# mumianyuxin/M3DSSD

Measured on AMD Instinct MI355X. Metric: images/sec at 1280x384 bs=8, 1/2/4/8 MI355X; 3D-box Linf vs ref, higher is better.
Workload: dtype f32; 1 GPU; BASELINE.json configs[1]: full M3d_inference_align (DLA-34 + DCNv2 align + ANAB) forward + decode + top-3000 + NMS, bs=8/GPU, 1280x384, fp32, random-init synthetic weights and frames; per_gpu_batch=8, global_batch=8, parallelism=dp1 (batch sharded, 1 all-gather of [B,40,14] detections)

## Files before the change

### include/m3dssd_hip.h

```cpp
#ifndef M3DSSD_HIP_H
#define M3DSSD_HIP_H

#include <stdint.h>

#ifdef __cplusplus
extern "C" {
#endif

typedef void *m3d_stream_t;

enum {
    M3D_OK = 0,
    M3D_E_ARG = -1,
    M3D_E_HIP = -2,
    M3D_E_WORKSPACE = -3
};

const char *m3d_last_error(void);
#define M3D_ABI_VERSION 5
int m3d_abi_version(void);
const char *m3d_source_hashes(void);

typedef struct m3d_conv_desc {
    const float *in;
// ... 15 lines not shown
    int res_mode;
    int act;
    int sigmoid_from;
    const float *dcn_offmask;
    int dcn_om_cs;
    float *splitk_ws;
    long long splitk_ws_bytes;
} m3d_conv_desc;

int m3d_conv2d_forward(const m3d_conv_desc *d, m3d_stream_t stream);
int m3d_conv2d_splitk_plan(const m3d_conv_desc *d, int *splits, long long *ws_bytes);

int m3d_conv_wave_applicable(const m3d_conv_desc *d);
int m3d_conv_wave_splitk_plan(const m3d_conv_desc *d, int *splits, long long *ws_bytes);
int m3d_conv_wave_forward(const m3d_conv_desc *d, m3d_stream_t stream);

int m3d_wino_conv3x3_forward(const m3d_conv_desc *d, m3d_stream_t stream);
int m3d_wino_conv3x3_variant(const m3d_conv_desc *d);
int m3d_wino_conv3x3_splitk_plan(const m3d_conv_desc *d, int *splits, long long *ws_bytes);
int m3d_wino_conv3x3_forward_ex(const m3d_conv_desc *d, int variant, m3d_stream_t stream);
int m3d_wino44_applicable(const m3d_conv_desc *d);
int m3d_wino44_conv3x3_forward(const m3d_conv_desc *d, m3d_stream_t stream);
int m3d_wino44_conv3x3_forward_ex(const m3d_conv_desc *d, int nb, m3d_stream_t stream);
int m3d_wino44_kpair(const m3d_conv_desc *d);
int m3d_wino44_splitk_plan(const m3d_conv_desc *d, int *splits, long long *ws_bytes);
int m3d_wino44_conv3x3_forward_touch(const m3d_conv_desc *d, int nb, const void *touch, long long touch_bytes, m3d_stream_t stream);

int m3d_cache_touch(const void *p, long long bytes, m3d_stream_t stream);
int m3d_upload_indirect(const void *const *src_slot, void *dst, long long bytes, m3d_stream_t stream);

// ... 315 lines not shown
```

### m3dssd_amd/_hip.py

```python
import ctypes
import os
import subprocess

_HERE = os.path.dirname(os.path.abspath(__file__))
CSRC = os.path.join(_HERE, "csrc")
SO_PATH = os.environ.get("M3D_HIP_LIB") or os.path.join(CSRC, "build", "libm3dssd_hip.so")
HEADER = os.path.join(os.path.dirname(_HERE), "include", "m3dssd_hip.h")

c_int, c_float, c_ll, c_void_p = ctypes.c_int, ctypes.c_float, ctypes.c_longlong, ctypes.c_void_p


class ConvDesc(ctypes.Structure):
    _fields_ = [
        ("inp", c_void_p), ("in_cs", c_int),
        ("N", c_int), ("H", c_int), ("W", c_int), ("Cin", c_int),
        ("wgt", c_void_p), ("wgt_img_stride", c_ll),
        ("Cout", c_int), ("Cout_pad", c_int),
        ("kh", c_int), ("kw", c_int), ("stride", c_int), ("pad", c_int), ("dil", c_int),
        ("Ho", c_int), ("Wo", c_int),
        ("out", c_void_p), ("out_cs", c_int), ("out_nchw", c_int), ("out_img_stride", c_ll),
        ("scale", c_void_p), ("shift", c_void_p),
        ("res", c_void_p), ("res_cs", c_int), ("res_mode", c_int),
        ("act", c_int), ("sigmoid_from", c_int),
        ("dcn_offmask", c_void_p), ("dcn_om_cs", c_int),
# ... 111 lines not shown
    "m3d_wino_conv3x3_forward": (c_int, [ctypes.POINTER(ConvDesc), P]),
    "m3d_wino_conv3x3_forward_ex": (c_int, [ctypes.POINTER(ConvDesc), c_int, P]),
    "m3d_wino_conv3x3_splitk_plan": (c_int, [ctypes.POINTER(ConvDesc), ctypes.POINTER(c_int), ctypes.POINTER(c_ll)]),
    "m3d_wino_conv3x3_variant": (c_int, [ctypes.POINTER(ConvDesc)]),
    "m3d_wino44_applicable": (c_int, [ctypes.POINTER(ConvDesc)]),
    "m3d_wino44_conv3x3_forward": (c_int, [ctypes.POINTER(ConvDesc), P]),
    "m3d_wino44_conv3x3_forward_ex": (c_int, [ctypes.POINTER(ConvDesc), c_int, P]),
    "m3d_wino44_kpair": (c_int, [ctypes.POINTER(ConvDesc)]),
    "m3d_wino44_conv3x3_forward_touch": (c_int, [ctypes.POINTER(ConvDesc), c_int, P, c_ll, P]),
    "m3d_cache_touch": (c_int, [P, c_ll, P]),
    "m3d_upload_indirect": (c_int, [P, P, c_ll, P]),
    "m3d_wino44_splitk_plan": (c_int, [ctypes.POINTER(ConvDesc), ctypes.POINTER(c_int), ctypes.POINTER(c_ll)]),
    "m3d_conv_wave_applicable": (c_int, [ctypes.POINTER(ConvDesc)]),
    "m3d_conv_wave_splitk_plan": (c_int, [ctypes.POINTER(ConvDesc), ctypes.POINTER(c_int), ctypes.POINTER(c_ll)]),
    "m3d_conv_wave_forward": (c_int, [ctypes.POINTER(ConvDesc), P]),
    "m3d_conv2d_tile": (c_int, [ctypes.POINTER(ConvDesc)] + [ctypes.POINTER(c_int)] * 4),
    "m3d_conv2d_splitk_plan": (c_int, [ctypes.POINTER(ConvDesc), ctypes.POINTER(c_int), ctypes.POINTER(c_ll)]),
    "m3d_dcn_v2_workspace_bytes": (c_ll, [c_int] * 10),
    "m3d_dcn_v2_workspace_bytes_grouped": (c_ll, [c_int] * 11),
    "m3d_dcn_v2_forward": (c_int, [P] * 6 + [c_int] * 14 + [P, c_ll, P]),
    "m3d_dcn_v2_backward_workspace_bytes": (c_ll, [c_int] * 11),
    "m3d_dcn_v2_backward": (c_int, [P] * 10 + [c_int] * 14 + [P, c_ll, P]),
    "m3d_rpn_loss_workspace_bytes": (c_ll, [c_int, c_ll]),
    "m3d_rpn_targets": (c_int, [P, c_int, c_int, c_int, P, c_int, P, c_int, c_int, P, P, c_int, P, P, P, P, P, c_ll, P]),
    "m3d_rpn_loss": (c_int, [P, c_int, c_int, c_int, P, c_int, P, c_int, c_int, P, P, P, c_int, P, P, P, P, P, P, P, P, P, P, c_ll, P]),
    "m3d_pack_conv_weight": (c_int, [P, P] + [c_int] * 6 + [P]),
    "m3d_nchw_to_nhwc": (c_int, [P, P] + [c_int] * 5 + [P]),
    "m3d_nhwc_to_nchw": (c_int, [P, c_int, P] + [c_int] * 4 + [P]),
    "m3d_stem_conv7x7": (c_int, [P, P, P, P, P] + [c_int] * 4 + [P]),
    "m3d_refine_3d": (c_int, [P, P, c_int, c_int, P, P, ctypes.c_double, c_int, ctypes.c_double, ctypes.c_double, P, P]),
# ... 92 lines not shown
```

### m3dssd_amd/csrc/common.h

```cpp
#pragma once
#include <hip/hip_runtime.h>
#include <stdarg.h>
#include <stdio.h>

#include "m3dssd_hip.h"

typedef float f32x4 __attribute__((ext_vector_type(4)));
typedef float f32x16 __attribute__((ext_vector_type(16)));
typedef float f32x2 __attribute__((ext_vector_type(2)));
typedef unsigned u32x4 __attribute__((ext_vector_type(4)));

__device__ __forceinline__ int sign_smear(int x)
{
    int m;
    asm("v_ashrrev_i32 %0, 31, %1" : "=v"(m) : "v"(x));
    return m;
}
__device__ __forceinline__ void dcn_corners(float h_im, float w_im, int H, int W, int drop_all, float (&w)[4], int (&o)[4],
                                            int (&drop)[4])
{
    const float tin = fminf(fminf(h_im, w_im) + 1.f, -fmaxf(h_im - (float)H, w_im - (float)W));
    const unsigned xin = __float_as_uint(tin);
    const unsigned nonfinite = __float_as_uint((h_im - h_im) + (w_im - w_im)) & 0x7fffffffu;
    const int out = sign_smear((int)((xin - 1u) | xin)) | sign_smear(-(int)nonfinite) | drop_all;
// ... 91 lines not shown
    do {                                                                            \
        hipError_t e__ = hipGetLastError();                                         \
        if (e__ != hipSuccess) {                                                    \
            m3d_set_error("kernel launch failed: %s (%s:%d)", hipGetErrorString(e__), \
                          __FILE__, __LINE__);                                      \
            return M3D_E_HIP;                                                       \
        }                                                                           \
    } while (0)

static inline int cdiv(long long a, long long b) { return (int)((a + b - 1) / b); }
static inline int imin(int a, int b) { return a < b ? a : b; }

__device__ __forceinline__ float leaky(float v) { return fmaxf(v, v * M3D_LEAKY_SLOPE); }
__device__ __forceinline__ float sigmoidf_(float v) { return 1.0f / (1.0f + expf(-v)); }

__device__ __forceinline__ f32x4 class_softmax4(f32x4 l)
{
    const float mx = fmaxf(fmaxf(l[0], l[1]), fmaxf(l[2], l[3]));
    f32x4 e;
    float s = 0.f;
#pragma unroll
    for (int c = 0; c < 4; ++c) { e[c] = expf(l[c] - mx); s += e[c]; }
    f32x4 pr;
#pragma unroll
    for (int c = 0; c < 4; ++c) pr[c] = e[c] / s;
    return pr;
}
__device__ __forceinline__ float fg_score(f32x4 pr) { return fmaxf(fmaxf(pr[1], pr[2]), pr[3]); }
__device__ __forceinline__ unsigned int f32_sortable(float f)
{
// ... 11 lines not shown
```

### m3dssd_amd/csrc/dcn_wave.hip

```cpp
#include <stdlib.h>

#include <type_traits>

#include "common.h"

struct ConvWaveArgs {
    const float *in, *wfrag, *scale, *shift, *res, *om;
    float *out;
    int in_cs, out_cs, res_cs, om_cs;
    int H, W, Cin, Ho, Wo, HoWo, Cout;
    int kh, kw, stride, pad, dil;
    int M, KG, tiles_n;
    int act, res_mode, sigmoid_from;
    int vec_out;
    long long w_img_stride;
    unsigned in_bytes, out_bytes, res_bytes, w_bytes;
    float *ws;
    int splits, ss_per, base_waves;
    unsigned ws_bytes;
#ifdef CONV_TRACE
    long long *trace;
#endif
};


#ifdef CONV_TRACE
static long long *g_conv_trace = nullptr;
extern "C" void m3d_conv_wave_set_trace(void *buf) { g_conv_trace = (long long *)buf; }
static int g_conv_variant = 0;
extern "C" void m3d_conv_wave_set_variant(int v) { g_conv_variant = v; }
#define TRACE_INIT() long long *trp = a.trace ? a.trace + (size_t)blockIdx.x * 128 : nullptr; int tri = 0
#define TRACE() do { if (trp && lane == 0 && tri < 128) trp[tri++] = __builtin_readcyclecounter(); } while (0)
#else
#define TRACE_INIT()
#define TRACE()
#endif

template <bool DEFORM, int NT, int NCQ = 4, int WPE = (DEFORM ? 2 : 3)>
__global__ __launch_bounds__(64) __attribute__((amdgpu_waves_per_eu(WPE))) void conv_wave_kernel(const ConvWaveArgs a)
{
    __shared__ __attribute__((aligned(16))) float tileA[32 * 32];
    __shared__ __attribute__((aligned(16))) float tapst[(DEFORM ? 9 : 1) * 32 * 8];
    const int lane = threadIdx.x, l31 = lane & 31, h = lane >> 5;
    const int gp = lane >> 3, gc = lane & 7;
    TRACE_INIT();
    TRACE();
    int blk;
    {
        const int nblk = gridDim.x, bid = blockIdx.x;
        const int q = nblk >> 3, r = nblk & 7, xcd = bid & 7, loc = bid >> 3;
        blk = (xcd < r ? xcd * (q + 1) : r * (q + 1) + (xcd - r) * q) + loc;
    }
    int split = 0;
    if (a.splits > 1) {
        split = blk / a.base_waves;
        blk -= split * a.base_waves;
    }
    const int bm = blk / a.tiles_n, bn = blk - bm * a.tiles_n;
    const int m0 = bm * 32;
    const int KK = a.kh * a.kw, C32 = a.Cin / 32;
    const int ss0 = split * a.ss_per, ss1 = min(KK * C32, ss0 + a.ss_per);

    const __amdgpu_buffer_rsrc_t rin = make_rsrc(a.in, a.in_bytes);
    const __amdgpu_buffer_rsrc_t rw =
        make_rsrc(a.wfrag + (size_t)(m0 / a.HoWo) * a.w_img_stride + (size_t)bn * NT * a.KG * 256, a.w_bytes);
    const unsigned wlane = (unsigned)lane * 16u;
    const unsigned wstride = (unsigned)a.KG * 1024u;

    int o_pix = 0, o_hi0 = 0, o_wi0 = 0;
    bool o_valid = false;
    int o_inv = -1;
    const float *o_om = a.om;
    int g_pix[4], g_hi0[4], g_wi0[4];
    bool g_valid[4];
    {
        const int m = m0 + l31;
// ... 12 lines not shown
        for (int g = 0; g < 4; ++g) {
            const int m = m0 + 8 * g + gp;
            g_valid[g] = m < a.M;
            const int mm = g_valid[g] ? m : 0;
            const int n = mm / a.HoWo, rem = mm - n * a.HoWo;
            const int ho = rem / a.Wo, wo = rem - ho * a.Wo;
            g_pix[g] = n * a.H * a.W;
            g_hi0[g] = ho * a.stride - a.pad;
            g_wi0[g] = wo * a.stride - a.pad;
        }
    }

    unsigned doff[4][DEFORM ? 4 : 1];
    float bw[DEFORM ? 4 : 1][4];
    if constexpr (DEFORM) {
        float raws[9][3];
#pragma unroll
        for (int t = 0; t < 9; ++t) {
            const int tp = min(t, KK - 1);
            raws[t][0] = o_om[2 * tp];
            raws[t][1] = o_om[2 * tp + 1];
            raws[t][2] = o_om[2 * KK + tp];
        }
#pragma unroll
        for (int t = 0; t < 9; ++t) {
            if (t < KK) {
                const int ti = t / a.kw, tj = t - ti * a.kw;
                const float mk = raws[t][2];
                const float h_im = (float)(o_hi0 + ti * a.dil) + raws[t][0];
                const float w_im = (float)(o_wi0 + tj * a.dil) + raws[t][1];
                float wq[4];
                int oq[4], drop[4];
                dcn_corners(h_im, w_im, a.H, a.W, o_inv, wq, oq, drop);
                u32x4 ob;
#pragma unroll
                for (int q = 0; q < 4; ++q) {
                    const unsigned off = ((unsigned)o_pix + (unsigned)oq[q]) * (unsigned)a.in_cs * 4u;
                    ob[q] = (off & ~(unsigned)drop[q]) | (M3D_BUF_OOB & (unsigned)drop[q]);
                }
                if (h == 0) {
                    *reinterpret_cast<u32x4 *>(&tapst[t * 256 + l31 * 8]) = ob;
                    *reinterpret_cast<f32x4 *>(&tapst[t * 256 + l31 * 8 + 4]) = f32x4{wq[0] * mk, wq[1] * mk, wq[2] * mk, wq[3] * mk};
                }
            }
        }
    }
    auto setup_tap = [&](int tap) {
        if constexpr (DEFORM) {
#pragma unroll
            for (int g = 0; g < 4; ++g) {
                const u32x4 ov = *reinterpret_cast<const u32x4 *>(&tapst[tap * 256 + (8 * g + gp) * 8]);
                const f32x4 wv = *reinterpret_cast<const f32x4 *>(&tapst[tap * 256 + (8 * g + gp) * 8 + 4]);
#pragma unroll
                for (int q = 0; q < 4; ++q) {
                    doff[g][q] = ov[q] + (unsigned)gc * 16u;
                    bw[g][q] = wv[q];
                }
            }
        } else {
            const int ti = tap / a.kw, tj = tap - ti * a.kw;
// ... 89 lines not shown
                for (int nt = 0; nt < NT; ++nt)
                    acc[nt] = __builtin_amdgcn_mfma_f32_32x32x2f32(A[j][t], bf[nt][t], acc[nt], 0, 0, 0);
            __builtin_amdgcn_sched_barrier(0);
        };
        group(0, kg0 + 1, bfA, bfB);
        group(1, kg0 + 2, bfB, bfA);
        group(2, kg0 + 3, bfA, bfB);
        group(3, kgn, bfB, bfA);
    }

    TRACE();
    const __amdgpu_buffer_rsrc_t rout = make_rsrc(a.out, a.out_bytes);
    const __amdgpu_buffer_rsrc_t rres = make_rsrc(a.res ? a.res : a.out, a.res ? a.res_bytes : 0u);
    const int n0 = bn * 32 * NT;
    const int mb = m0 + 4 * h;
    if (a.splits > 1) {
        const __amdgpu_buffer_rsrc_t rws = make_rsrc(a.ws, a.ws_bytes);
        const unsigned sbase = (unsigned)split * (unsigned)a.M;
        const unsigned cpad = (unsigned)(a.tiles_n * 32 * NT);
#pragma unroll
        for (int nt = 0; nt < NT; ++nt) {
            const unsigned co = (unsigned)(n0 + nt * 32 + l31);
#pragma unroll
            for (int r = 0; r < 16; ++r) {
                const int m = mb + (r & 3) + 8 * (r >> 2);
                const unsigned oo = m < a.M ? ((sbase + (unsigned)m) * cpad + co) * 4u : M3D_BUF_OOB;
                const float pv = acc[nt][r];
                __builtin_amdgcn_raw_buffer_store_b32(__builtin_bit_cast(unsigned, pv), rws, oo, 0, 0);
            }
        }
// ... 38 lines not shown
                        rv[q] = __builtin_bit_cast(f32x4, __builtin_amdgcn_raw_buffer_load_b128(rres, rq[q] + (unsigned)c * 4u, 0, 0));
                    } else {
#pragma unroll
                        for (int e = 0; e < 4; ++e)
                            rv[q][e] = __builtin_bit_cast(float, __builtin_amdgcn_raw_buffer_load_b32(
                                rres, c + e < a.Cout ? rq[q] + (unsigned)(c + e) * 4u : M3D_BUF_OOB, 0, 0));
                    }
                }
            }
#pragma unroll
            for (int r = 0; r < 16; ++r) tileA[((r & 3) + 8 * (r >> 2) + 4 * h) * 32 + l31] = acc[nt][r];
            const bool tile_sig = a.sigmoid_from >= 0 && n0 + nt * 32 + 31 >= a.sigmoid_from;
#pragma unroll
            for (int q = 0; q < 4; ++q) {
                f32x4 v = *reinterpret_cast<const f32x4 *>(&tileA[(pr + 8 * q) * 32 + 4 * c4]);
                if (a.res) v = a.res_mode ? (v + rv[q]) * scv[nt] + shv[nt] : v * scv[nt] + shv[nt] + rv[q];
                else v = v * scv[nt] + shv[nt];
                if (tile_sig) {
#pragma unroll
                    for (int e = 0; e < 4; ++e) v[e] = c + e >= a.sigmoid_from ? sigmoidf_(v[e]) : fmaxf(v[e], v[e] * slope);
                } else {
                    v = __builtin_elementwise_max(v, v * slope);
                }
                if (c + 3 < a.Cout) {
                    __builtin_amdgcn_raw_buffer_store_b128(__builtin_bit_cast(u32x4, v), rout, oq[q] + (unsigned)c * 4u, 0, 0);
                } else {
#pragma unroll
                    for (int e = 0; e < 4; ++e)
                        __builtin_amdgcn_raw_buffer_store_b32(__builtin_bit_cast(unsigned, v[e]), rout,
                                                              c + e < a.Cout ? oq[q] + (unsigned)(c + e) * 4u : M3D_BUF_OOB, 0, 0);
                }
            }
        }
        TRACE();
        return;
    }
#pragma unroll
    for (int nt = 0; nt < NT; ++nt) {
        const int co = n0 + nt * 32 + l31;
        const bool cok = co < a.Cout;
        const float sc = (cok && a.scale) ? a.scale[co] : 1.f;
        const float sh = (cok && a.shift) ? a.shift[co] : 0.f;
        float rv[16];
        if (a.res) {
#pragma unroll
            for (int r = 0; r < 16; ++r) {
                const int m = mb + (r & 3) + 8 * (r >> 2);
                const unsigned ro = (cok && m < a.M) ? ((unsigned)m * (unsigned)a.res_cs + (unsigned)co) * 4u : M3D_BUF_OOB;
                rv[r] = __builtin_bit_cast(float, __builtin_amdgcn_raw_buffer_load_b32(rres, ro, 0, 0));
            }
        }
#pragma unroll
        for (int r = 0; r < 16; ++r) {
            const int m = mb + (r & 3) + 8 * (r >> 2);
            float v = acc[nt][r];
            if (a.res) v = a.res_mode ? (v + rv[r]) * sc + sh : v * sc + sh + rv[r];
            else v = v * sc + sh;
            if (a.sigmoid_from >= 0 && co >= a.sigmoid_from) v = sigmoidf_(v);
            else if (a.act == 1) v = fmaxf(v, v * M3D_LEAKY_SLOPE);
            const unsigned oo = (cok && m < a.M) ? ((unsigned)m * (unsigned)a.out_cs + (unsigned)co) * 4u : M3D_BUF_OOB;
            __builtin_amdgcn_raw_buffer_store_b32(__builtin_bit_cast(unsigned, v), rout, oo, 0, 0);
        }
    }
    TRACE();
}

static int conv_wave_plan(const m3d_conv_desc *d, bool enforce_min, int *splits, int *ss_per)
{
    *splits = 1;
    *ss_per = d->kh * d->kw * (d->Cin / 32);
    if (d->out_nchw) return 0;
    if (d->dcn_offmask && d->kh * d->kw > 9) return 0;
    if (d->Cin % 32 != 0 || d->Cout_pad % 64 != 0) return 0;
    const int cw = d->Cout_pad % 128 == 0 ? 128 : 64;
    if (d->wgt_img_stride && (d->Ho * d->Wo) % 32 != 0) return 0;
    const long long M = (long long)d->N * d->Ho * d->Wo;
    const long long base = ((M + 31) / 32) * (d->Cout_pad / cw);
    if (base >= (1ll << 28)) return 0;
    static int wave_min = -1, dcn_min = -1, splitk = -1;
    if (wave_min < 0) { const char *e = getenv("M3D_CONV_WAVE_MIN"); wave_min = e ? atoi(e) : 900; }
    if (dcn_min < 0) { const char *e = getenv("M3D_DCN_WAVE_MIN"); dcn_min = e ? atoi(e) : 1500; }
    if (splitk < 0) { const char *e = getenv("M3D_CONV_WAVE_SPLITK"); splitk = e ? atoi(e) : 1; }
    const long long need = d->dcn_offmask ? dcn_min : wave_min;
    const int nss = *ss_per;
    if (base < need && splitk && d->splitk_ws) {
        int s = (int)((1800 + base - 1) / base);
        if (s > nss / 4) s = nss / 4;
        if (s > 8) s = 8;
        if (s >= 2) {
// ... 6 lines not shown
}

extern "C" int m3d_conv_wave_applicable(const m3d_conv_desc *d)
{
    int s, p;
    return d ? conv_wave_plan(d, true, &s, &p) : 0;
}

extern "C" int m3d_conv_wave_splitk_plan(const m3d_conv_desc *d, int *splits, long long *ws_bytes)
{
    M3D_REQUIRE(d && splits && ws_bytes, "conv_wave_splitk_plan: null pointer");
    m3d_conv_desc t = *d;
    static float dummy;
    t.splitk_ws = &dummy;
    int p;
    const int waves = conv_wave_plan(&t, true, splits, &p);
    if (waves == 0) *splits = 1;
    *ws_bytes = *splits > 1 ? (long long)*splits * d->N * d->Ho * d->Wo * d->Cout_pad * 4 : 0;
    return M3D_OK;
}

extern "C" int m3d_conv_wave_forward(const m3d_conv_desc *d, m3d_stream_t stream_)
{
    hipStream_t stream = (hipStream_t)stream_;
    M3D_REQUIRE(d && d->in && d->wgt && d->out, "conv_wave: null pointer");
    int splits = 1, ss_per = 0;
    const int waves = conv_wave_plan(d, false, &splits, &ss_per);
    M3D_REQUIRE(waves > 0, "conv_wave: needs Cin %% 32 == 0, Cout_pad %% 64 == 0, NHWC output, Ho*Wo %% 32 == 0 with per-image weights");
    const int ho = (d->H + 2 * d->pad - (d->dil * (d->kh - 1) + 1)) / d->stride + 1;
    const int wo = (d->W + 2 * d->pad - (d->dil * (d->kw - 1) + 1)) / d->stride + 1;
    M3D_REQUIRE(ho == d->Ho && wo == d->Wo, "conv_wave: Ho/Wo mismatch");
    M3D_REQUIRE(d->in_cs % 32 == 0 && d->in_cs >= d->Cin && ((uintptr_t)d->in & 127) == 0 && ((uintptr_t)d->wgt & 15) == 0,
                "conv_wave: the input view must be 128-byte aligned with in_cs %% 32 == 0");
    const long long M = (long long)d->N * d->Ho * d->Wo;
    M3D_REQUIRE(!d->wgt_img_stride || (d->wgt_img_stride % 4 == 0 && d->stride == 1 && d->Ho == d->H && d->Wo == d->W),
                "conv_wave: per-image weights need an image-aligned 16-byte stride and a same-size output");
    M3D_REQUIRE((long long)d->N * d->H * d->W * d->in_cs * 4 < (1ll << 31) && M * d->out_cs * 4 < (1ll << 31) &&
                M * d->res_cs * 4 < (1ll << 31) && (long long)d->Cout_pad * d->kh * d->kw * d->Cin * 4 < (1ll << 31),
                "conv_wave: views must be < 2 GiB");
    ConvWaveArgs a;
    a.in = d->in; a.wfrag = d->wgt; a.scale = d->scale; a.shift = d->shift; a.res = d->res; a.om = d->dcn_offmask;
    a.out = d->out;
    a.in_cs = d->in_cs; a.out_cs = d->out_cs; a.res_cs = d->res_cs; a.om_cs = d->dcn_om_cs;
    a.H = d->H; a.W = d->W; a.Cin = d->Cin; a.Ho = d->Ho; a.Wo = d->Wo; a.HoWo = d->Ho * d->Wo; a.Cout = d->Cout;
    a.kh = d->kh; a.kw = d->kw; a.stride = d->stride; a.pad = d->pad; a.dil = d->dil;
    const int cw = d->Cout_pad % 128 == 0 ? 128 : 64;
    a.M = (int)M; a.KG = d->kh * d->kw * d->Cin / 8; a.tiles_n = d->Cout_pad / cw;
    a.act = d->act; a.res_mode = d->res_mode; a.sigmoid_from = d->sigmoid_from; a.w_img_stride = d->wgt_img_stride;
    static int vec_epi = -1;
    if (vec_epi < 0) { const char *e = getenv("M3D_WAVE_VEC_EPILOGUE"); vec_epi = e ? atoi(e) : 1; }
    a.vec_out = vec_epi && d->out_cs % 4 == 0 && ((uintptr_t)d->out & 15) == 0 &&
                (!d->res || (d->res_cs % 4 == 0 && ((uintptr_t)d->res & 15) == 0)) &&
                (!d->scale || ((uintptr_t)d->scale & 15) == 0) && (!d->shift || ((uintptr_t)d->shift & 15) == 0);
    a.in_bytes = (unsigned)((long long)d->N * d->H * d->W * d->in_cs * 4);
    a.out_bytes = (unsigned)(M * d->out_cs * 4);
    a.res_bytes = (unsigned)(M * d->res_cs * 4);
    a.w_bytes = (unsigned)((long long)cw * d->kh * d->kw * d->Cin * 4);
#ifdef CONV_TRACE
    a.trace = g_conv_trace;
#endif
    a.ws = nullptr; a.splits = 1; a.ss_per = ss_per; a.base_waves = waves; a.ws_bytes = 0;
    if (splits > 1) {
        const long long need = (long long)splits * M * d->Cout_pad * 4;
        M3D_REQUIRE(need <= d->splitk_ws_bytes && need < (1ll << 31) && ((uintptr_t)d->splitk_ws & 15) == 0,
                    "conv_wave: split-K workspace too small (%lld bytes, see m3d_conv_wave_splitk_plan), >= 2 GiB or misaligned",
                    d->splitk_ws_bytes);
        a.ws = d->splitk_ws; a.splits = splits; a.base_waves = waves / splits; a.ws_bytes = (unsigned)need;
    }
#ifdef CONV_TRACE
    if (g_conv_variant && d->dcn_offmask && cw == 128) {
        switch (g_conv_variant) {
        case 1: hipLaunchKernelGGL((conv_wave_kernel<true, 4, 1, 2>), dim3(waves), dim3(64), 0, stream, a); break;
        case 2: hipLaunchKernelGGL((conv_wave_kernel<true, 4, 1, 3>), dim3(waves), dim3(64), 0, stream, a); break;
        case 3: hipLaunchKernelGGL((conv_wave_kernel<true, 4, 2, 2>), dim3(waves), dim3(64), 0, stream, a); break;
        case 4: hipLaunchKernelGGL((conv_wave_kernel<true, 4, 2, 3>), dim3(waves), dim3(64), 0, stream, a); break;
        default: hipLaunchKernelGGL((conv_wave_kernel<true, 4, 4, 3>), dim3(waves), dim3(64), 0, stream, a); break;
        }
        M3D_LAUNCH_CHECK();
        return M3D_OK;
    }
#endif
    if (cw == 128) {
        if (d->dcn_offmask) hipLaunchKernelGGL((conv_wave_kernel<true, 4>), dim3(waves), dim3(64), 0, stream, a);
        else hipLaunchKernelGGL((conv_wave_kernel<false, 4>), dim3(waves), dim3(64), 0, stream, a);
    } else {
        if (d->dcn_offmask) hipLaunchKernelGGL((conv_wave_kernel<true, 2>), dim3(waves), dim3(64), 0, stream, a);
        else hipLaunchKernelGGL((conv_wave_kernel<false, 2>), dim3(waves), dim3(64), 0, stream, a);
    }
    M3D_LAUNCH_CHECK();
    if (splits > 1) {
        SplitkReduceArgs r;
        r.ws = a.ws; r.scale = d->scale; r.shift = d->shift; r.res = d->res; r.out = d->out;
        r.M = (int)M; r.Cout = d->Cout; r.Cout_pad = d->Cout_pad; r.splits = splits; r.out_cs = d->out_cs; r.res_cs = d->res_cs;
        r.res_mode = d->res_mode; r.act = d->act; r.sigmoid_from = d->sigmoid_from;
        return m3d_launch_splitk_reduce(r, stream);
    }
    return M3D_OK;
}
```

### m3dssd_amd/csrc/igemm_conv.hip

```cpp
#include <stdlib.h>

#include "common.h"

#ifdef IGEMM_TRACE
#define IG_ABL(bit) (a.ablate & (bit))
#else
#define IG_ABL(bit) false
#endif

struct IgemmArgs {
    const float *in;
    const float *wgt;
    float *out;
    const float *scale;
    const float *shift;
    const float *res;
    const float *om;
    const float *zero;
    long long wgt_img_stride;
    long long out_img_stride;
    int in_cs, out_cs, res_cs, om_cs;
    int H, W, Cin, Ho, Wo, HoWo;
    int Cout, Cout_pad;
    int kh, kw, stride, pad, dil;
// ... 310 lines not shown
        }
    }
}

__global__ __launch_bounds__(256) void splitk_reduce_kernel(const SplitkReduceArgs a, int vec_out)
{
    const int c4n = a.Cout_pad >> 2;
    const long long i = (long long)blockIdx.x * 256 + threadIdx.x;
    if (i >= (long long)a.M * c4n) return;
    const int m = (int)(i / c4n), co0 = (int)(i - (long long)m * c4n) * 4;
    if (co0 >= a.Cout) return;
    const size_t stride = (size_t)a.M * a.Cout_pad;
    const float *p = a.ws + (size_t)m * a.Cout_pad + co0;
    f32x4 v = *reinterpret_cast<const f32x4 *>(p);
    for (int s = 1; s < a.splits; ++s) v = v + *reinterpret_cast<const f32x4 *>(p + s * stride);
    f32x4 o;
#pragma unroll
    for (int q = 0; q < 4; ++q) {
        const int co = co0 + q;
        float x = v[q];
        if (co < a.Cout) {
            const float sc = a.scale ? a.scale[co] : 1.f;
            const float sh = a.shift ? a.shift[co] : 0.f;
            if (a.res) {
                const float rv = a.res[(size_t)m * a.res_cs + co];
                x = a.res_mode ? (x + rv) * sc + sh : x * sc + sh + rv;
            } else {
                x = x * sc + sh;
            }
            if (a.sigmoid_from >= 0 && co >= a.sigmoid_from) x = sigmoidf_(x);
            else if (a.act == 1) x = leaky(x);
        }
        o[q] = x;
    }
    float *op = a.out + (size_t)m * a.out_cs + co0;
    if (vec_out && co0 + 3 < a.Cout) {
        *reinterpret_cast<f32x4 *>(op) = o;
    } else {
#pragma unroll
        for (int q = 0; q < 4; ++q)
            if (co0 + q < a.Cout) op[q] = o[q];
    }
}

int m3d_launch_splitk_reduce(const SplitkReduceArgs &a, hipStream_t stream)
{
// ... 196 lines not shown
```

### m3dssd_amd/engine.py

```python
import ctypes
import math
import os

import numpy as np
import torch

from . import _hip
from ._hip import ConvDesc, MlpDesc
from .config import model_flags

BN_EPS = 1e-5
SELECT_KEYS = os.environ.get("M3D_SELECT_KEYS", "1") != "0"
PSP_SIZES = (1, 4, 8, 16)
BACKBONE_CHANNELS = {"dla34": (16, 32, 64, 128, 256, 512), "dla102": (16, 32, 128, 256, 512, 1024)}
DLA102_LEVELS = (1, 1, 1, 3, 4, 1)


def _rup(a, b):
    return (a + b - 1) // b * b


class View:
    __slots__ = ("t", "ptr", "n", "h", "w", "c", "cs", "keep")

# ... 101 lines not shown


def pack_wino44_c16(weight, device):
    g = weight.detach().to("cpu", torch.float64)
    assert tuple(g.shape) == (16, 16, 3, 3)
    u = torch.einsum("ai,ocij,bj->abco", _WINO44_G, g, _WINO44_G).reshape(36, 4, 4, 16)
    return u.permute(0, 1, 3, 2).contiguous().to(torch.float32).reshape(-1).to(device)


WINO_MIN_BLOCKS = int(os.environ.get("M3D_WINO_MIN_BLOCKS", "128"))
FUSED_ANAB = os.environ.get("M3D_FUSED_ANAB", "1") != "0"
USE_ANAB_WAVE = os.environ.get("M3D_ANAB_WAVE", "1") != "0"
USE_ANAB_NESTED = os.environ.get("M3D_ANAB_NESTED", "1") != "0"
USE_DCN_WAVE = os.environ.get("M3D_DCN_WAVE", "1") != "0"
USE_CONV_WAVE = os.environ.get("M3D_CONV_WAVE", "1") != "0"
USE_WINO = os.environ.get("M3D_WINO", "1") != "0"
USE_WINO44 = os.environ.get("M3D_WINO44", "1") != "0"
WINO44_TOUCH = os.environ.get("M3D_WINO44_TOUCH", "1") != "0"
WINO44_TOUCH_SPAN = int(os.environ.get("M3D_WINO44_TOUCH_SPAN", "2"))
USE_WINO44_SPLITK = os.environ.get("M3D_WINO44_SPLITK", "1") != "0"
W44_SPLIT_NB = 2 if os.environ.get("M3D_W44_SPLIT_NB", "1") == "2" else 1
W44_SPLIT_KPAIR = os.environ.get("M3D_W44_SPLIT_NB", "1") == "3"
WINO44_MIN_WGS = int(os.environ.get("M3D_WINO44_MIN_WGS", "1000000"))
WINO44_MIN_WGS_NB1 = int(os.environ.get("M3D_WINO44_MIN_WGS_NB1", "200"))


class OpCost:

    def __init__(self, hbm_bytes):
        self.hbm_bytes = int(hbm_bytes)
# ... 268 lines not shown
                kind = "wino_lds<64,32,16>"
            plan.ops.append((name, kind, flops, lambda st: _hip.check(L.m3d_wino_conv3x3_forward(ref, st)), d))
            return
        flops_true = 2.0 * x.n * d.Ho * d.Wo * d.Cout * kh * kw * (
            cin_true if cin_true is not None else (pc.cin if (pc is not None and wgt_ptr is None) else x.c))
        if wgt_frag:
            assert wgt_ptr is not None and planar is None and x.cs % 32 == 0 and x.ptr % 128 == 0, name
            if L.m3d_conv_wave_applicable(ref) <= 0:
                raise RuntimeError("%s: fragment-ordered weights but the wave kernel does not apply" % name)
            plan.ops.append((name, "conv_wave", flops_true, lambda st: _hip.check(L.m3d_conv_wave_forward(ref, st)), d))
            return
        if (pc is not None and wgt_ptr is None and planar is None and (USE_DCN_WAVE if om is not None else USE_CONV_WAVE)
                and x.cs % 32 == 0 and x.ptr % 128 == 0 and pc.cin_pad == x.c):
            wsplits, wbytes = ctypes.c_int(), ctypes.c_longlong()
            _hip.check(L.m3d_conv_wave_splitk_plan(ref, ctypes.byref(wsplits), ctypes.byref(wbytes)))
            ws = None
            if wsplits.value > 1:
                ws = torch.empty(wbytes.value // 4, device=self.device, dtype=torch.float32)
                d.splitk_ws, d.splitk_ws_bytes = ws.data_ptr(), wbytes.value
            if L.m3d_conv_wave_applicable(ref) > 0:
                frag = pc.frag()
                d.wgt = frag.data_ptr()
                if ws is not None:
                    plan.keep.append(ws)
                kind = "conv_wave%s" % ("<%s>" % ",".join(
                    (["deform"] if om is not None else []) + (["splitk%d" % wsplits.value] if wsplits.value > 1 else []))
                    if (om is not None or wsplits.value > 1) else "")
                plan.ops.append((name, kind, flops_true, lambda st: _hip.check(L.m3d_conv_wave_forward(ref, st)), d))
                return
            d.splitk_ws, d.splitk_ws_bytes = None, 0
        bm, bn, bk, grid = ctypes.c_int(), ctypes.c_int(), ctypes.c_int(), ctypes.c_int()
        _hip.check(L.m3d_conv2d_tile(ref, ctypes.byref(bm), ctypes.byref(bn), ctypes.byref(bk), ctypes.byref(grid)))
# ... 546 lines not shown
```

Measured before the change: 1373 images/sec.

## Reduce split-K conv slices inside one workgroup via LDS instead of global workspace

```diff
diff --git a/include/m3dssd_hip.h b/include/m3dssd_hip.h
--- a/include/m3dssd_hip.h
+++ b/include/m3dssd_hip.h
@@ -53,6 +53,8 @@
 int m3d_conv_wave_applicable(const m3d_conv_desc *d);
 int m3d_conv_wave_splitk_plan(const m3d_conv_desc *d, int *splits, long long *ws_bytes);
 int m3d_conv_wave_forward(const m3d_conv_desc *d, m3d_stream_t stream);
+int m3d_conv_wave_forward_wgsplit(const m3d_conv_desc *d, m3d_stream_t stream);
+int m3d_conv_wave_wgsplit_width(const m3d_conv_desc *d, int *slices, int *width);
 
 int m3d_wino_conv3x3_forward(const m3d_conv_desc *d, m3d_stream_t stream);
 int m3d_wino_conv3x3_variant(const m3d_conv_desc *d);
diff --git a/m3dssd_amd/_hip.py b/m3dssd_amd/_hip.py
--- a/m3dssd_amd/_hip.py
+++ b/m3dssd_amd/_hip.py
@@ -149,6 +149,8 @@
     "m3d_conv_wave_applicable": (c_int, [ctypes.POINTER(ConvDesc)]),
     "m3d_conv_wave_splitk_plan": (c_int, [ctypes.POINTER(ConvDesc), ctypes.POINTER(c_int), ctypes.POINTER(c_ll)]),
     "m3d_conv_wave_forward": (c_int, [ctypes.POINTER(ConvDesc), P]),
+    "m3d_conv_wave_forward_wgsplit": (c_int, [ctypes.POINTER(ConvDesc), P]),
+    "m3d_conv_wave_wgsplit_width": (c_int, [ctypes.POINTER(ConvDesc), ctypes.POINTER(c_int), ctypes.POINTER(c_int)]),
     "m3d_conv2d_tile": (c_int, [ctypes.POINTER(ConvDesc)] + [ctypes.POINTER(c_int)] * 4),
     "m3d_conv2d_splitk_plan": (c_int, [ctypes.POINTER(ConvDesc), ctypes.POINTER(c_int), ctypes.POINTER(c_ll)]),
     "m3d_dcn_v2_workspace_bytes": (c_ll, [c_int] * 10),
diff --git a/m3dssd_amd/csrc/common.h b/m3dssd_amd/csrc/common.h
--- a/m3dssd_amd/csrc/common.h
+++ b/m3dssd_amd/csrc/common.h
@@ -129,6 +129,23 @@
 __device__ __forceinline__ float leaky(float v) { return fmaxf(v, v * M3D_LEAKY_SLOPE); }
 __device__ __forceinline__ float sigmoidf_(float v) { return 1.0f / (1.0f + expf(-v)); }
 
+template <typename T>
+__device__ __forceinline__ T conv_epi_affine(T v, T sc, T sh, T rv, bool has_res, int res_mode)
+{
+    if (has_res) return res_mode ? (v + rv) * sc + sh : v * sc + sh + rv;
+    return v * sc + sh;
+}
+__device__ __forceinline__ float conv_epi_act(float v, bool sig, float slope) { return sig ? sigmoidf_(v) : fmaxf(v, v * slope); }
+__device__ __forceinline__ f32x4 conv_epi_act4(f32x4 v, int c0, int sigmoid_from, bool any_sig, float slope)
+{
+    if (any_sig) {
+#pragma unroll
+        for (int e = 0; e < 4; ++e) v[e] = conv_epi_act(v[e], c0 + e >= sigmoid_from, slope);
+        return v;
+    }
+    return __builtin_elementwise_max(v, v * slope);
+}
+
 __device__ __forceinline__ f32x4 class_softmax4(f32x4 l)
 {
     const float mx = fmaxf(fmaxf(l[0], l[1]), fmaxf(l[2], l[3]));
diff --git a/m3dssd_amd/csrc/dcn_wave.hip b/m3dssd_amd/csrc/dcn_wave.hip
--- a/m3dssd_amd/csrc/dcn_wave.hip
+++ b/m3dssd_amd/csrc/dcn_wave.hip
@@ -29,19 +29,21 @@
 extern "C" void m3d_conv_wave_set_trace(void *buf) { g_conv_trace = (long long *)buf; }
 static int g_conv_variant = 0;
 extern "C" void m3d_conv_wave_set_variant(int v) { g_conv_variant = v; }
-#define TRACE_INIT() long long *trp = a.trace ? a.trace + (size_t)blockIdx.x * 128 : nullptr; int tri = 0
+#define TRACE_INIT() long long *trp = (a.trace && threadIdx.x < 64) ? a.trace + (size_t)blockIdx.x * 128 : nullptr; int tri = 0
 #define TRACE() do { if (trp && lane == 0 && tri < 128) trp[tri++] = __builtin_readcyclecounter(); } while (0)
 #else
 #define TRACE_INIT()
 #define TRACE()
 #endif
 
-template <bool DEFORM, int NT, int NCQ = 4, int WPE = (DEFORM ? 2 : 3)>
-__global__ __launch_bounds__(64) __attribute__((amdgpu_waves_per_eu(WPE))) void conv_wave_kernel(const ConvWaveArgs a)
-{
-    __shared__ __attribute__((aligned(16))) float tileA[32 * 32];
+template <bool DEFORM, int NT, int NCQ = 4, int WPE = (DEFORM ? 2 : 3), int S = 1>
+__global__ __launch_bounds__(64 * S) __attribute__((amdgpu_waves_per_eu(WPE))) void conv_wave_kernel(const ConvWaveArgs a)
+{
+    __shared__ __attribute__((aligned(16))) float tileS[S * 32 * 32];
     __shared__ __attribute__((aligned(16))) float tapst[(DEFORM ? 9 : 1) * 32 * 8];
-    const int lane = threadIdx.x, l31 = lane & 31, h = lane >> 5;
+    const int lane = threadIdx.x & 63, l31 = lane & 31, h = lane >> 5;
+    const int wv = S > 1 ? __builtin_amdgcn_readfirstlane((int)threadIdx.x >> 6) : 0;
+    float *const tileA = tileS + wv * 1024;
     const int gp = lane >> 3, gc = lane & 7;
     TRACE_INIT();
     TRACE();
@@ -51,15 +53,16 @@
         const int q = nblk >> 3, r = nblk & 7, xcd = bid & 7, loc = bid >> 3;
         blk = (xcd < r ? xcd * (q + 1) : r * (q + 1) + (xcd - r) * q) + loc;
     }
-    int split = 0;
-    if (a.splits > 1) {
+    int split = wv;
+    if (S == 1 && a.splits > 1) {
         split = blk / a.base_waves;
         blk -= split * a.base_waves;
     }
     const int bm = blk / a.tiles_n, bn = blk - bm * a.tiles_n;
     const int m0 = bm * 32;
     const int KK = a.kh * a.kw, C32 = a.Cin / 32;
-    const int ss0 = split * a.ss_per, ss1 = min(KK * C32, ss0 + a.ss_per);
+    const bool idle = S > 1 && wv >= a.splits;
+    const int ss0 = idle ? 0 : split * a.ss_per, ss1 = idle ? 0 : min(KK * C32, ss0 + a.ss_per);
 
     const __amdgpu_buffer_rsrc_t rin = make_rsrc(a.in, a.in_bytes);
     const __amdgpu_buffer_rsrc_t rw =
@@ -102,21 +105,23 @@
     unsigned doff[4][DEFORM ? 4 : 1];
     float bw[DEFORM ? 4 : 1][4];
     if constexpr (DEFORM) {
-        float raws[9][3];
-#pragma unroll
-        for (int t = 0; t < 9; ++t) {
-            const int tp = min(t, KK - 1);
-            raws[t][0] = o_om[2 * tp];
-            raws[t][1] = o_om[2 * tp + 1];
-            raws[t][2] = o_om[2 * KK + tp];
-        }
-#pragma unroll
-        for (int t = 0; t < 9; ++t) {
+        constexpr int TPW = (9 + S - 1) / S;
+        float raws[TPW][3];
+#pragma unroll
+        for (int i = 0; i < TPW; ++i) {
+            const int tp = min(wv + i * S, KK - 1);
+            raws[i][0] = o_om[2 * tp];
+            raws[i][1] = o_om[2 * tp + 1];
+            raws[i][2] = o_om[2 * KK + tp];
+        }
+#pragma unroll
+        for (int i = 0; i < TPW; ++i) {
+            const int t = wv + i * S;
             if (t < KK) {
                 const int ti = t / a.kw, tj = t - ti * a.kw;
-                const float mk = raws[t][2];
-                const float h_im = (float)(o_hi0 + ti * a.dil) + raws[t][0];
-                const float w_im = (float)(o_wi0 + tj * a.dil) + raws[t][1];
+                const float mk = raws[i][2];
+                const float h_im = (float)(o_hi0 + ti * a.dil) + raws[i][0];
+                const float w_im = (float)(o_wi0 + tj * a.dil) + raws[i][1];
                 float wq[4];
                 int oq[4], drop[4];
                 dcn_corners(h_im, w_im, a.H, a.W, o_inv, wq, oq, drop);
@@ -132,6 +137,7 @@
                 }
             }
         }
+        if constexpr (S > 1) __syncthreads();
     }
     auto setup_tap = [&](int tap) {
         if constexpr (DEFORM) {
@@ -251,6 +257,89 @@
     const __amdgpu_buffer_rsrc_t rres = make_rsrc(a.res ? a.res : a.out, a.res ? a.res_bytes : 0u);
     const int n0 = bn * 32 * NT;
     const int mb = m0 + 4 * h;
+    if constexpr (S > 1) {
+        constexpr int Q = S == 2 ? 2 : 1;
+        const int tid = threadIdx.x;
+        const bool worker = S < 8 || wv < 4;
+        const float slope = a.act == 1 ? M3D_LEAKY_SLOPE : 1.f;
+        const int c4 = lane & 7;
+        int px[Q];
+        unsigned oq[Q], rq[Q];
+#pragma unroll
+        for (int q = 0; q < Q; ++q) {
+            px[q] = ((tid + q * 64 * S) >> 3) & 31;
+            const int m = m0 + px[q];
+            const bool ok = worker && m < a.M;
+            oq[q] = ok ? (unsigned)m * (unsigned)a.out_cs * 4u : M3D_BUF_OOB;
+            rq[q] = ok ? (unsigned)m * (unsigned)a.res_cs * 4u : M3D_BUF_OOB;
+        }
+        f32x4 scv[NT], shv[NT];
+#pragma unroll
+        for (int nt = 0; nt < NT; ++nt) {
+            const int c = n0 + nt * 32 + 4 * c4;
+            scv[nt] = f32x4{1.f, 1.f, 1.f, 1.f};
+            shv[nt] = f32x4{0.f, 0.f, 0.f, 0.f};
+            if (a.vec_out && c + 3 < a.Cout) {
+                if (a.scale) scv[nt] = *reinterpret_cast<const f32x4 *>(a.scale + c);
+                if (a.shift) shv[nt] = *reinterpret_cast<const f32x4 *>(a.shift + c);
+            } else {
+#pragma unroll
+                for (int e = 0; e < 4; ++e)
+                    if (c + e < a.Cout) {
+                        if (a.scale) scv[nt][e] = a.scale[c + e];
+                        if (a.shift) shv[nt][e] = a.shift[c + e];
+                    }
+            }
+        }
+#pragma unroll
+        for (int nt = 0; nt < NT; ++nt) {
+            const int c = n0 + nt * 32 + 4 * c4;
+            const bool full = a.vec_out && c + 3 < a.Cout;
+            f32x4 rv[Q];
+            if (a.res) {
+#pragma unroll
+                for (int q = 0; q < Q; ++q) {
+                    if (full) {
+                        rv[q] = __builtin_bit_cast(f32x4, __builtin_amdgcn_raw_buffer_load_b128(rres, rq[q] + (unsigned)c * 4u, 0, 0));
+                    } else {
+#pragma unroll
+                        for (int e = 0; e < 4; ++e)
+                            rv[q][e] = __builtin_bit_cast(float, __builtin_amdgcn_raw_buffer_load_b32(
+                                rres, c + e < a.Cout ? rq[q] + (unsigned)(c + e) * 4u : M3D_BUF_OOB, 0, 0));
+                    }
+                }
+            }
+            if (nt) __syncthreads();
+#pragma unroll
+            for (int r = 0; r < 16; ++r) tileA[((r & 3) + 8 * (r >> 2) + 4 * h) * 32 + l31] = acc[nt][r];
+            __syncthreads();
+            if (worker) {
+                const bool tile_sig = a.sigmoid_from >= 0 && n0 + nt * 32 + 31 >= a.sigmoid_from;
+#pragma unroll
+                for (int q = 0; q < Q; ++q) {
+                    const float *p = &tileS[px[q] * 32 + 4 * c4];
+                    f32x4 v = *reinterpret_cast<const f32x4 *>(p);
+#pragma unroll
+                    for (int s = 1; s < S; ++s)
+                        if (s < a.splits) v = v + *reinterpret_cast<const f32x4 *>(p + s * 1024);
+                    v = conv_epi_affine(v, scv[nt], shv[nt], a.res ? rv[q] : v, a.res != nullptr, a.res_mode);
+                    v = conv_epi_act4(v, c, a.sigmoid_from, tile_sig, slope);
+                    if (full) {
+                        __builtin_amdgcn_raw_buffer_store_b128(__builtin_bit_cast(u32x4, v), rout, oq[q] + (unsigned)c * 4u, 0, 0);
+                    } else {
+#pragma unroll
+                        for (int e = 0; e < 4; ++e) {
+                            const float pe = v[e];
+                            __builtin_amdgcn_raw_buffer_store_b32(__builtin_bit_cast(unsigned, pe), rout,
+                                                                  c + e < a.Cout ? oq[q] + (unsigned)(c + e) * 4u : M3D_BUF_OOB, 0, 0);
+                        }
+                    }
+                }
+            }
+        }
+        TRACE();
+        return;
+    }
     if (a.splits > 1) {
         const __amdgpu_buffer_rsrc_t rws = make_rsrc(a.ws, a.ws_bytes);
         const unsigned sbase = (unsigned)split * (unsigned)a.M;
@@ -319,21 +408,17 @@
 #pragma unroll
             for (int q = 0; q < 4; ++q) {
                 f32x4 v = *reinterpret_cast<const f32x4 *>(&tileA[(pr + 8 * q) * 32 + 4 * c4]);
-                if (a.res) v = a.res_mode ? (v + rv[q]) * scv[nt] + shv[nt] : v * scv[nt] + shv[nt] + rv[q];
-                else v = v * scv[nt] + shv[nt];
-                if (tile_sig) {
-#pragma unroll
-                    for (int e = 0; e < 4; ++e) v[e] = c + e >= a.sigmoid_from ? sigmoidf_(v[e]) : fmaxf(v[e], v[e] * slope);
-                } else {
-                    v = __builtin_elementwise_max(v, v * slope);
-                }
+                v = conv_epi_affine(v, scv[nt], shv[nt], a.res ? rv[q] : v, a.res != nullptr, a.res_mode);
+                v = conv_epi_act4(v, c, a.sigmoid_from, tile_sig, slope);
                 if (c + 3 < a.Cout) {
                     __builtin_amdgcn_raw_buffer_store_b128(__builtin_bit_cast(u32x4, v), rout, oq[q] + (unsigned)c * 4u, 0, 0);
                 } else {
 #pragma unroll
-                    for (int e = 0; e < 4; ++e)
-                        __builtin_amdgcn_raw_buffer_store_b32(__builtin_bit_cast(unsigned, v[e]), rout,
+                    for (int e = 0; e < 4; ++e) {
+                        const float pe = v[e];
+                        __builtin_amdgcn_raw_buffer_store_b32(__builtin_bit_cast(unsigned, pe), rout,
                                                               c + e < a.Cout ? oq[q] + (unsigned)(c + e) * 4u : M3D_BUF_OOB, 0, 0);
+                    }
                 }
             }
         }
@@ -358,11 +443,8 @@
 #pragma unroll
         for (int r = 0; r < 16; ++r) {
             const int m = mb + (r & 3) + 8 * (r >> 2);
-            float v = acc[nt][r];
-            if (a.res) v = a.res_mode ? (v + rv[r]) * sc + sh : v * sc + sh + rv[r];
-            else v = v * sc + sh;
-            if (a.sigmoid_from >= 0 && co >= a.sigmoid_from) v = sigmoidf_(v);
-            else if (a.act == 1) v = fmaxf(v, v * M3D_LEAKY_SLOPE);
+            float v = conv_epi_affine(acc[nt][r], sc, sh, a.res ? rv[r] : 0.f, a.res != nullptr, a.res_mode);
+            v = conv_epi_act(v, a.sigmoid_from >= 0 && co >= a.sigmoid_from, a.act == 1 ? M3D_LEAKY_SLOPE : 1.f);
             const unsigned oo = (cok && m < a.M) ? ((unsigned)m * (unsigned)a.out_cs + (unsigned)co) * 4u : M3D_BUF_OOB;
             __builtin_amdgcn_raw_buffer_store_b32(__builtin_bit_cast(unsigned, v), rout, oo, 0, 0);
         }
@@ -370,14 +452,15 @@
     TRACE();
 }
 
-static int conv_wave_plan(const m3d_conv_desc *d, bool enforce_min, int *splits, int *ss_per)
+static int conv_wave_plan(const m3d_conv_desc *d, bool enforce_min, int *splits, int *ss_per, bool allow32 = false)
 {
     *splits = 1;
     *ss_per = d->kh * d->kw * (d->Cin / 32);
     if (d->out_nchw) return 0;
     if (d->dcn_offmask && d->kh * d->kw > 9) return 0;
-    if (d->Cin % 32 != 0 || d->Cout_pad % 64 != 0) return 0;
-    const int cw = d->Cout_pad % 128 == 0 ? 128 : 64;
+    if (d->Cin % 32 != 0 || d->Cout_pad % 32 != 0) return 0;
+    if (d->Cout_pad % 64 != 0 && (!allow32 || d->dcn_offmask || d->wgt_img_stride)) return 0;
+    const int cw = d->Cout_pad % 128 == 0 ? 128 : (d->Cout_pad % 64 == 0 ? 64 : 32);
     if (d->wgt_img_stride && (d->Ho * d->Wo) % 32 != 0) return 0;
     const long long M = (long long)d->N * d->Ho * d->Wo;
     const long long base = ((M + 31) / 32) * (d->Cout_pad / cw);
@@ -414,19 +497,34 @@
     static float dummy;
     t.splitk_ws = &dummy;
     int p;
-    const int waves = conv_wave_plan(&t, true, splits, &p);
+    const int waves = conv_wave_plan(&t, true, splits, &p, true);
     if (waves == 0) *splits = 1;
-    *ws_bytes = *splits > 1 ? (long long)*splits * d->N * d->Ho * d->Wo * d->Cout_pad * 4 : 0;
+    *ws_bytes = (*splits > 1 && d->Cout_pad % 64 == 0) ? (long long)*splits * d->N * d->Ho * d->Wo * d->Cout_pad * 4 : 0;
     return M3D_OK;
 }
 
-extern "C" int m3d_conv_wave_forward(const m3d_conv_desc *d, m3d_stream_t stream_)
-{
-    hipStream_t stream = (hipStream_t)stream_;
-    M3D_REQUIRE(d && d->in && d->wgt && d->out, "conv_wave: null pointer");
+template <bool DEFORM, int NT>
+static void launch_wgsplit(const ConvWaveArgs &a, int S, int wgs, hipStream_t stream)
+{
+    constexpr int WPE = DEFORM ? 2 : 3;
+    switch (S) {
+    case 2: hipLaunchKernelGGL((conv_wave_kernel<DEFORM, NT, 4, WPE, 2>), dim3(wgs), dim3(128), 0, stream, a); break;
+    case 4: hipLaunchKernelGGL((conv_wave_kernel<DEFORM, NT, 4, WPE, 4>), dim3(wgs), dim3(256), 0, stream, a); break;
+    default: hipLaunchKernelGGL((conv_wave_kernel<DEFORM, NT, 4, WPE, 8>), dim3(wgs), dim3(512), 0, stream, a); break;
+    }
+}
+
+static int conv_wave_run(const m3d_conv_desc *d_, hipStream_t stream, bool wgsplit)
+{
+    M3D_REQUIRE(d_ && d_->in && d_->wgt && d_->out, "conv_wave: null pointer");
+    m3d_conv_desc dd = *d_;
+    static float dummy;
+    if (wgsplit) { dd.splitk_ws = &dummy; dd.splitk_ws_bytes = 0; }
+    const m3d_conv_desc *d = &dd;
     int splits = 1, ss_per = 0;
-    const int waves = conv_wave_plan(d, false, &splits, &ss_per);
-    M3D_REQUIRE(waves > 0, "conv_wave: needs Cin %% 32 == 0, Cout_pad %% 64 == 0, NHWC output, Ho*Wo %% 32 == 0 with per-image weights");
+    const int waves = conv_wave_plan(d, false, &splits, &ss_per, wgsplit);
+    M3D_REQUIRE(waves > 0, "conv_wave: needs Cin %% 32 == 0, Cout_pad %% 64 == 0 (%% 32: plain, shared weights, wgsplit entry), NHWC output, "
+                           "Ho*Wo %% 32 == 0 with per-image weights");
     const int ho = (d->H + 2 * d->pad - (d->dil * (d->kh - 1) + 1)) / d->stride + 1;
     const int wo = (d->W + 2 * d->pad - (d->dil * (d->kw - 1) + 1)) / d->stride + 1;
     M3D_REQUIRE(ho == d->Ho && wo == d->Wo, "conv_wave: Ho/Wo mismatch");
@@ -444,7 +542,7 @@
     a.in_cs = d->in_cs; a.out_cs = d->out_cs; a.res_cs = d->res_cs; a.om_cs = d->dcn_om_cs;
     a.H = d->H; a.W = d->W; a.Cin = d->Cin; a.Ho = d->Ho; a.Wo = d->Wo; a.HoWo = d->Ho * d->Wo; a.Cout = d->Cout;
     a.kh = d->kh; a.kw = d->kw; a.stride = d->stride; a.pad = d->pad; a.dil = d->dil;
-    const int cw = d->Cout_pad % 128 == 0 ? 128 : 64;
+    const int cw = d->Cout_pad % 128 == 0 ? 128 : (d->Cout_pad % 64 == 0 ? 64 : 32);
     a.M = (int)M; a.KG = d->kh * d->kw * d->Cin / 8; a.tiles_n = d->Cout_pad / cw;
     a.act = d->act; a.res_mode = d->res_mode; a.sigmoid_from = d->sigmoid_from; a.w_img_stride = d->wgt_img_stride;
     static int vec_epi = -1;
@@ -460,6 +558,22 @@
     a.trace = g_conv_trace;
 #endif
     a.ws = nullptr; a.splits = 1; a.ss_per = ss_per; a.base_waves = waves; a.ws_bytes = 0;
+    if (splits > 1 && wgsplit) {
+        const int S = splits <= 2 ? 2 : (splits <= 4 ? 4 : 8);
+        M3D_REQUIRE(splits <= 8, "conv_wave: %d K slices do not fit a workgroup", splits);
+        a.splits = splits; a.base_waves = waves / splits;
+        if (cw == 128) {
+            if (d->dcn_offmask) launch_wgsplit<true, 4>(a, S, a.base_waves, stream);
+            else launch_wgsplit<false, 4>(a, S, a.base_waves, stream);
+        } else if (cw == 64) {
+            if (d->dcn_offmask) launch_wgsplit<true, 2>(a, S, a.base_waves, stream);
+            else launch_wgsplit<false, 2>(a, S, a.base_waves, stream);
+        } else {
+            launch_wgsplit<false, 1>(a, S, a.base_waves, stream);
+        }
+        M3D_LAUNCH_CHECK();
+        return M3D_OK;
+    }
     if (splits > 1) {
         const long long need = (long long)splits * M * d->Cout_pad * 4;
         M3D_REQUIRE(need <= d->splitk_ws_bytes && need < (1ll << 31) && ((uintptr_t)d->splitk_ws & 15) == 0,
@@ -483,6 +597,8 @@
     if (cw == 128) {
         if (d->dcn_offmask) hipLaunchKernelGGL((conv_wave_kernel<true, 4>), dim3(waves), dim3(64), 0, stream, a);
         else hipLaunchKernelGGL((conv_wave_kernel<false, 4>), dim3(waves), dim3(64), 0, stream, a);
+    } else if (cw == 32) {
+        hipLaunchKernelGGL((conv_wave_kernel<false, 1>), dim3(waves), dim3(64), 0, stream, a);
     } else {
         if (d->dcn_offmask) hipLaunchKernelGGL((conv_wave_kernel<true, 2>), dim3(waves), dim3(64), 0, stream, a);
         else hipLaunchKernelGGL((conv_wave_kernel<false, 2>), dim3(waves), dim3(64), 0, stream, a);
@@ -497,3 +613,26 @@
     }
     return M3D_OK;
 }
+
+extern "C" int m3d_conv_wave_forward(const m3d_conv_desc *d, m3d_stream_t stream)
+{
+    return conv_wave_run(d, (hipStream_t)stream, false);
+}
+
+extern "C" int m3d_conv_wave_wgsplit_width(const m3d_conv_desc *d, int *slices, int *width)
+{
+    M3D_REQUIRE(d && slices && width, "conv_wave_wgsplit_width: null pointer");
+    m3d_conv_desc t = *d;
+    static float dummy;
+    t.splitk_ws = &dummy;
+    int p;
+    const int waves = conv_wave_plan(&t, false, slices, &p, true);
+    M3D_REQUIRE(waves > 0 && *slices <= 8, "conv_wave_wgsplit_width: the wave kernel does not apply to this descriptor");
+    *width = *slices <= 1 ? 1 : (*slices <= 2 ? 2 : (*slices <= 4 ? 4 : 8));
+    return M3D_OK;
+}
+
+extern "C" int m3d_conv_wave_forward_wgsplit(const m3d_conv_desc *d, m3d_stream_t stream)
+{
+    return conv_wave_run(d, (hipStream_t)stream, true);
+}
diff --git a/m3dssd_amd/csrc/igemm_conv.hip b/m3dssd_amd/csrc/igemm_conv.hip
--- a/m3dssd_amd/csrc/igemm_conv.hip
+++ b/m3dssd_amd/csrc/igemm_conv.hip
@@ -348,6 +348,7 @@
     const float *p = a.ws + (size_t)m * a.Cout_pad + co0;
     f32x4 v = *reinterpret_cast<const f32x4 *>(p);
     for (int s = 1; s < a.splits; ++s) v = v + *reinterpret_cast<const f32x4 *>(p + s * stride);
+    const float slope = a.act == 1 ? M3D_LEAKY_SLOPE : 1.f;
     f32x4 o;
 #pragma unroll
     for (int q = 0; q < 4; ++q) {
@@ -356,14 +357,9 @@
         if (co < a.Cout) {
             const float sc = a.scale ? a.scale[co] : 1.f;
             const float sh = a.shift ? a.shift[co] : 0.f;
-            if (a.res) {
-                const float rv = a.res[(size_t)m * a.res_cs + co];
-                x = a.res_mode ? (x + rv) * sc + sh : x * sc + sh + rv;
-            } else {
-                x = x * sc + sh;
-            }
-            if (a.sigmoid_from >= 0 && co >= a.sigmoid_from) x = sigmoidf_(x);
-            else if (a.act == 1) x = leaky(x);
+            const float rv = a.res ? a.res[(size_t)m * a.res_cs + co] : 0.f;
+            x = conv_epi_affine(x, sc, sh, rv, a.res != nullptr, a.res_mode);
+            x = conv_epi_act(x, a.sigmoid_from >= 0 && co >= a.sigmoid_from, slope);
         }
         o[q] = x;
     }
diff --git a/m3dssd_amd/engine.py b/m3dssd_amd/engine.py
--- a/m3dssd_amd/engine.py
+++ b/m3dssd_amd/engine.py
@@ -139,6 +139,8 @@
 USE_ANAB_NESTED = os.environ.get("M3D_ANAB_NESTED", "1") != "0"
 USE_DCN_WAVE = os.environ.get("M3D_DCN_WAVE", "1") != "0"
 USE_CONV_WAVE = os.environ.get("M3D_CONV_WAVE", "1") != "0"
+USE_CONV_WAVE_WGSPLIT = os.environ.get("M3D_CONV_WAVE_WGSPLIT", "1") != "0"
+USE_OFFMASK_WAVE = os.environ.get("M3D_OFFMASK_WAVE", "1") != "0"
 USE_WINO = os.environ.get("M3D_WINO", "1") != "0"
 USE_WINO44 = os.environ.get("M3D_WINO44", "1") != "0"
 WINO44_TOUCH = os.environ.get("M3D_WINO44_TOUCH", "1") != "0"
@@ -437,8 +439,14 @@
                 and x.cs % 32 == 0 and x.ptr % 128 == 0 and pc.cin_pad == x.c):
             wsplits, wbytes = ctypes.c_int(), ctypes.c_longlong()
             _hip.check(L.m3d_conv_wave_splitk_plan(ref, ctypes.byref(wsplits), ctypes.byref(wbytes)))
+            if wsplits.value > 1 and USE_CONV_WAVE_WGSPLIT and (d.Cout_pad % 64 == 0 or (USE_OFFMASK_WAVE and wsplits.value <= 4)):
+                frag = pc.frag()
+                d.wgt = frag.data_ptr()
+                kind = "conv_wave<%s>" % ",".join((["deform"] if om is not None else []) + ["wgsplit%d" % wsplits.value])
+                plan.ops.append((name, kind, flops_true, lambda st: _hip.check(L.m3d_conv_wave_forward_wgsplit(ref, st)), d))
+                return
             ws = None
-            if wsplits.value > 1:
+            if wsplits.value > 1 and wbytes.value > 0:
                 ws = torch.empty(wbytes.value // 4, device=self.device, dtype=torch.float32)
                 d.splitk_ws, d.splitk_ws_bytes = ws.data_ptr(), wbytes.value
             if L.m3d_conv_wave_applicable(ref) > 0:
```

After: 1400 images/sec (median of 6 runs). 1.02x the previous value.
